# latentnetworks/vimure

Hardware: AMD Instinct MI355X
Metric: CAVI iterations/sec (L=4 N=2000 M=200 K=2 synthetic, mutuality on) (higher is better)
Workload: dtype f64

## Files before the change

### vimure_amd/csrc/sweep_sl.h

```cpp
#ifndef VMR_SWEEP_SL_H
#define VMR_SWEEP_SL_H

#include "vmr_internal.h"
#include <functional>

#define SL_YM(e) ((e) & 0xfffffu)
#define SL_INR(e) (((e) >> 20) & 1u)
#define SL_X(e) ((e) >> 21)
#define SL_XMAX 2047u
#define SL_YM_ROWS (1u << 20)
#define SL_PF 8
#ifndef SL_PFW
#define SL_PFW 8
#endif
constexpr int sl_pf(int K) { return K <= 2 ? SL_PF : SL_PFW; }
#define SL_SLACK (64 * 64)

struct SlArgs {
  const unsigned* E; const unsigned* rs; const unsigned long long* ebase; const unsigned* perm;
  const unsigned* sy;
  const uint8_t* cls;
  const unsigned* Qt;
  const uint64_t* Rb; const unsigned* rq; const unsigned short* Rm; const unsigned long long* rbase;
  const unsigned* rm2;
  double* rho; const double* logpr;
  const double* par; double* slotR; const double* lutg; double* Hg; double* slotF; double* slotA;
  int Gl;
  int do_hist;
  int yt, hc;
  int sum_a;
  double* nu_acc; double* elbo_dev; int commit_nu;
  int nu_stale;
  unsigned long long* det;
  int lp0;
  int farl;
  double* h0s;
  const unsigned* x0p;
  int lv0r;
  const unsigned* Ez;
  int elbo_cur;
  const double* lpd; const double* lpb;
#ifdef SL_DEBUG
  unsigned long long* dbg_t;
#endif
};

struct SlShape { int tpb, yt, hc; size_t smem; };
struct SlUnit { SlArgs a; Geo g; int blk0, nblk; };

#ifndef SL_LIGHT_UPD_K
#define SL_LIGHT_UPD_K 2
#endif
constexpr bool sl_light(int K, bool elbo, bool allfull, bool update) { return !elbo && allfull && (K <= SL_LIGHT_UPD_K || (!update && K <= 4)); }
#ifndef SL_ELBO3_K
#define SL_ELBO3_K 2
#endif
#ifndef SL_ELBO3
#define SL_ELBO3 1
#endif
constexpr int sl_tpb_max(int K, bool elbo, bool allfull, bool update = true) {
  return elbo ? ((SL_ELBO3 && K <= SL_ELBO3_K) ? 768 : (K <= 4 ? 512 : 256)) : (sl_light(K, elbo, allfull, update) ? 1024 : (K <= 3 ? 768 : (K <= 7 ? 512 : 256)));
}
constexpr int sl_tpb_max_b(int K, bool elbo, bool allfull) { return elbo ? sl_tpb_max(K, true, allfull) : (K <= 2 ? 768 : (K <= 7 ? 512 : 256)); }
constexpr int sl_wpe_b(int K, bool elbo, bool allfull) { return elbo ? ((SL_ELBO3 && K <= SL_ELBO3_K) ? 3 : (K <= 4 ? 2 : 1)) : (K <= 2 ? 3 : (K <= 7 ? 2 : 1)); }
constexpr int sl_wpe(int K, bool elbo, bool allfull, bool update = true) {
  return elbo ? ((SL_ELBO3 && K <= SL_ELBO3_K) ? 3 : (K <= 4 ? 2 : 1)) : (sl_light(K, elbo, allfull, update) ? 4 : (K <= 3 ? 3 : (K <= 7 ? 2 : 1)));
}

static inline size_t sl_smem(const Geo& g, int yt, int hc, bool update, bool elbo, bool hist) {
  const size_t lb = (size_t)g.Mp * g.K * 8;
  return (update ? (size_t)yt * lb : 0) + (hist ? (size_t)hc * lb : 0) + (size_t)g.Mp * 8 * (update ? 2 : 1) +
         (size_t)g.W * 8 + 128 + (g.ml ? lb + (size_t)g.Mp * 8 : 0) + (size_t)(64 + (elbo ? 256 : 0)) * 8 + 16;
}

typedef int (*sl_launch_fn)(vmr_ctx* h, int mode, const SlShape& sh, SlArgs& a);
sl_launch_fn vmr_sl_launcher(int K);
typedef int (*sl_launch_batch_fn)(vmr_ctx* h, hipStream_t st, int mode, int allfull, const SlUnit* units, const int* blk_unit, int nblocks,
                                  int tpb, size_t smem);
sl_launch_batch_fn vmr_sl_batch_launcher(int K);

#define SP_LDS_MAX (160 * 1024)
SlShape sl_shape(const vmr_ctx* h, bool update, bool elbo, bool hist);
SlArgs sl_args(const vmr_ctx* h, const SlShape& sh, int do_hist, int sum_a = 0);
int sl_launch(vmr_ctx* h, int mode, const SlShape& sh, SlArgs& a);

typedef std::function<void(int l, const unsigned* rpl, unsigned* etmp, unsigned* etmp2)> SlFill;
int sl_place_entries(vmr_ctx* h, unsigned* rp, const std::vector<unsigned long long>& nl, unsigned* etmp_all, unsigned* etmp2_all, const SlFill* fill);
int sl_balance_layer(vmr_ctx* h, int l, unsigned long long eb, unsigned rows_near);
int sl_permute_u8(vmr_ctx* h, const uint8_t* in, uint8_t* out);
int sl_permute_u32(vmr_ctx* h, const unsigned* in, unsigned* out);
int sl_permute_rows(vmr_ctx* h, const double* in, double* out, bool to_pos);

#endif
```

### vimure_amd/csrc/sweep_sl.hip

```cpp
#include "sweep_sl.h"

#ifndef VMR_K
#error "compile with -DVMR_K=<number of categories>"
#endif
#ifndef SL_WPE
#define SL_WPE sl_wpe(2, false, true)
#endif

template <int K>
struct StepIn {
  double v[K];
  double w[K];
  unsigned cls, qt, tie;
  unsigned x0;
  unsigned e[sl_pf(K)];
};

template <int R> struct RC { static constexpr int value = R; };
template <class V> __device__ __forceinline__ const V* at_bytes(const V* p, unsigned off) {
  return reinterpret_cast<const V*>(reinterpret_cast<const char*>(p) + off);
}
template <class V> __device__ __forceinline__ V* at_bytes(V* p, unsigned off) {
  return reinterpret_cast<V*>(reinterpret_cast<char*>(p) + off);
}
__device__ __forceinline__ double rcp_nr2(double d) {
  double r = __builtin_amdgcn_rcp(d);
  r = fma(fma(-d, r, 1.0), r, r);
  return fma(fma(-d, r, 1.0), r, r);
}
#define SL_INL __attribute__((always_inline))
#ifndef SL_BATCH2
#define SL_BATCH2 8
#endif
template <int K> struct Batch { static constexpr int value = K <= 2 ? SL_BATCH2 : (K <= 4 ? 4 : 2); };

template <int K, bool UPDATE, bool ELBO, bool ALLFULL, bool STORE = true, bool DET = false, bool LPD = false>
__device__ __forceinline__ void sweep_body(const SlArgs& a, const Geo& g, const unsigned bx, const unsigned gx) {
  extern __shared__ __align__(16) unsigned char smem[];
  constexpr int PFK = sl_pf(K);
  constexpr bool LV0 = !UPDATE && !ELBO && !DET;
  constexpr bool LV0R = UPDATE && K >= 3;
  const int tid = threadIdx.x, lane = tid & 63, nthr = (int)blockDim.x;
  const int wv = __builtin_amdgcn_readfirstlane(tid >> 6), nw = nthr >> 6;
  const int Mp = g.Mp;
  const unsigned ytm = UPDATE ? (unsigned)a.yt * (unsigned)Mp : 0u;
  const unsigned hcm = a.do_hist ? (unsigned)a.hc * (unsigned)Mp : 0u;
  size_t off = 0;
  double* F = reinterpret_cast<double*>(smem + off); off += (size_t)ytm * K * 8;
  const int nHc = (int)hcm * K;
  double* Hc = reinterpret_cast<double*>(smem + off); off += (size_t)nHc * 8;
  double* Gth = reinterpret_cast<double*>(smem + off); off += (size_t)Mp * 8;
  double* Lth = reinterpret_cast<double*>(smem + off); off += UPDATE ? (size_t)Mp * 8 : 0;
  double* As = reinterpret_cast<double*>(smem + off); off += a.sum_a ? (size_t)Mp * K * 8 : 0;
  double* wsum = reinterpret_cast<double*>(smem + off); off += (size_t)g.W * 8;
  double* red = reinterpret_cast<double*>(smem + off); off += 16 * 8;
  double* xt = reinterpret_cast<double*>(smem + off); off += 64 * 8;
  double* lt = reinterpret_cast<double*>(smem + off); off += ELBO ? 256 * 8 : 0;
  double* EthL = reinterpret_cast<double*>(smem + off); off += a.rq ? (size_t)Mp * 8 : 0;
  const ParOff o = par_off(g.L, g.Mp, g.K);
// ... 44 lines not shown
  unsigned long long ie_lin = 0ull, ie_q = 0ull, ie_log = 0ull, iaccF[K];
#pragma unroll
  for (int k = 0; k < K; ++k) iaccF[k] = 0ull;
  double* Hl = a.Hg + ((size_t)l * NH + (gb % NH)) * g.Y * Mp * K;
  auto det_H = [&]() SL_INL { return a.det + (size_t)l * g.Y * Mp * K; };
  auto det_A = [&]() SL_INL { return a.det + (size_t)g.L * g.Y * Mp * K + (size_t)l * g.W * 64 * K; };
  auto det_F = [&]() SL_INL { return a.det + (size_t)g.L * g.Y * Mp * K + (size_t)g.L * g.W * 64 * K + (size_t)l * K; };
  auto det_R = [&]() SL_INL { return a.det + (size_t)g.L * g.Y * Mp * K + (size_t)g.L * g.W * 64 * K + (size_t)g.L * K; };
  const unsigned* rsl = a.rs + (size_t)l * (NS + 1);
  const unsigned* syl = a.sy + (size_t)l * NS;
  const unsigned* El = a.E + a.ebase[l];
  const unsigned* pl = (a.rm2 ? a.rm2 : a.perm) + (size_t)l * NS * 64;
  const uint8_t* cl = ALLFULL ? nullptr : a.cls + (size_t)l * T;
  const unsigned* Ql = a.Qt ? a.Qt + (size_t)l * T : nullptr;
  const uint64_t* Rl = a.Rb ? a.Rb + (size_t)l * T * g.W : nullptr;
  double* rl = a.rho + (size_t)l * T * K;
  double* rho_slack = a.rho + (size_t)g.L * T * K;
  const double* lpl = a.logpr + (size_t)l * T * K;
  constexpr bool LPDV = LPD && K == 2 && UPDATE && !ELBO;
  const double* lpdl = LPDV ? a.lpd + (size_t)l * T : nullptr;
  const double lpb0 = (K == 2 && UPDATE) ? a.lpb[2 * l] : 0.0, lpb1 = (K == 2 && UPDATE) ? a.lpb[2 * l + 1] : 0.0;
  const unsigned* rql = a.rq ? a.rq + (size_t)l * (T + 1) : nullptr;
  const unsigned short* Rml = a.rq ? a.Rm + a.rbase[l] : nullptr;
  const unsigned lim_y = UPDATE ? (a.do_hist ? (unsigned)min(a.yt, a.hc) : (unsigned)a.yt) : (a.do_hist ? (unsigned)a.hc : 0xffffffffu);
  const unsigned lim1 = (UPDATE && a.yt < g.Y) ? (unsigned)a.yt : 0xffffffffu;
  const unsigned lim2 = (a.do_hist && a.hc < g.Y) ? (unsigned)a.hc : 0xffffffffu;

  const long long Gl_ = a.Gl;
  unsigned* tick = reinterpret_cast<unsigned*>(smem + off); off += 16;
  if (tid == 0) { tick[0] = 2u * (unsigned)nw; tick[1] = 0u; }
  auto step_of = [&](unsigned t) SL_INL -> long long { return (long long)gb + (long long)t * Gl_; };
  auto draw = [&]() SL_INL -> long long {
    unsigned t = 0u;
    if (lane == 0) t = atomicAdd(tick, 1u);
    return step_of((unsigned)__builtin_amdgcn_readfirstlane((int)t));
  };
  long long s = step_of((unsigned)wv), sn = step_of((unsigned)(nw + wv));
  unsigned ea = 0;
  int R = 0;
  unsigned ymax = 0;
  unsigned rgv = 0;
  StepIn<K> P;

  const unsigned lane4 = (unsigned)lane * 4u, laneK8 = (unsigned)lane * (unsigned)(K * 8);
  const unsigned T32 = (unsigned)T;
  auto fetch_range = [&](long long st) SL_INL {
    const unsigned ra = rsl[st + (lane < 1 ? 0 : 1)], ry = syl[st];
    rgv = lane == 2 ? ry : ra;
  };
  auto fetch_tie = [&](StepIn<K>& d, long long st, const bool lp_const = false) SL_INL {
    const size_t row0 = (size_t)st * 64;
    const bool ok = (unsigned)row0 + (unsigned)lane < T32;
    d.qt = 0u; d.tie = 0u;
// ... 31 lines not shown
    R = (int)((rsl[s + 1] - ea) >> 6);
    ymax = syl[s];
    fetch_range(sn < NS ? sn : s);
    fetch_tie(P, s);
    fetch_ent(P, ea, RC<PFK>{});
  }
#ifdef SL_DEBUG
  if (dbt && lane == 0) dbt[4] = wall_clock64();
#endif
  __builtin_amdgcn_s_waitcnt(0x0F70);
  bool lv0_off = false;
  if (LV0 || LV0R) lv0_off = __syncthreads_or(gz ? 1 : 0) != 0;
  else __syncthreads();
#ifdef SL_DEBUG
  if (dbt && lane == 0) dbt[5] = wall_clock64();
#endif
  const double gnu_f = a.par[o.sc + (a.nu_stale ? SC_G_NU_STALE : SC_G_NU)];
  if (UPDATE) {
    for (int q = tid; q < (int)ytm; q += nthr) {
      const int y = q / Mp, m = q - y * Mp;
#pragma unroll
      for (int k = 0; k < K; ++k) F[q * K + k] = (m < g.M) ? f_entry(g.mut, Lth[m], Gth[m], Lla[k], Gla[k], gnu_f, y) : 0.0;
    }
    __syncthreads();
  }
  double Tfull = 0.0;
  for (int w = 0; w < g.W; ++w) Tfull += wsum[w];
#ifdef SL_DEBUG
  if (dbt && lane == 0) dbt[1] = wall_clock64();
#endif

  auto add_lists = [&](unsigned t, bool on, const double (&rr)[K]) SL_INL {
    if (a.rm2) {
#pragma unroll
      for (int h_ = 0; h_ < 2; ++h_) {
        const unsigned m = h_ ? (t >> 16) : (t & 0xffffu);
        const bool v = on && m != 0xffffu;
        const unsigned long long vm = __ballot(v);
        if (vm == 0ull) continue;
        const int m0 = __builtin_amdgcn_readlane((int)m, __builtin_ctzll(vm));
        if (__all(!v || (int)m == m0)) {
#pragma unroll
          for (int k = 0; k < K; ++k) {
            const double sm_ = wave_sum(v ? rr[k] : 0.0);
            if (lane == 0) lds_add(&As[m0 * K + k], sm_, sc_a);
          }
        } else if (v) {
#pragma unroll
// ... 42 lines not shown
    }
    return Tt;
  };
  const double gnu_cur = a.par[o.sc + SC_G_NU];
  auto w2_at = [&](unsigned ym, int k) SL_INL -> double {
    const unsigned y = row_level(ym);
    const double z2 = gnu_cur * (double)y, den = Gth[ym - y * (unsigned)Mp] * Gla[k] + z2;
    return (y == 0u || den == 0.0) ? 0.0 : z2 / den;
  };
  auto f_far = [&](unsigned ym, double (&f)[K]) SL_INL {
    const unsigned y = row_level(ym);
    const unsigned m = ym - y * (unsigned)Mp;
    const double lt = Lth[m], gt = Gth[m];
#pragma unroll
    for (int k = 0; k < K; ++k) f[k] = f_entry(g.mut, lt, gt, Lla[k], Gla[k], gnu_f, (int)y);
  };
  auto elbo_inner = [&](unsigned ent, const double (&er)[2]) SL_INL -> double {
    const unsigned ym = SL_YM(ent);
    const unsigned y = row_level(ym);
    const double z2 = gnu * (double)y, gt = Gth[ym - y * (unsigned)Mp];
    const double inner = fma(gt, er[0], z2 * er[1]);
    return (SL_INR(ent) ? inner : 0.0) + eps;
  };
  auto walk1_near = [&](const unsigned* e, auto npc, double (&U)[K]) SL_INL {
    constexpr int NP = decltype(npc)::value, BT = Batch<K>::value;
#pragma unroll
    for (int j0 = 0; j0 < NP; j0 += BT) {
      double f[BT][K];
#pragma unroll
      for (int u = 0; u < BT; ++u) {
        if (j0 + u < NP) {
#pragma unroll
          for (int k = 0; k < K; ++k) f[u][k] = F[SL_YM(e[j0 + u]) * K + k];
        }
      }
#pragma unroll
      for (int u = 0; u < BT; ++u) {
        if (j0 + u < NP) {
          const double dx = (double)SL_X(e[j0 + u]);
#pragma unroll
          for (int k = 0; k < K; ++k) U[k] = fma(dx, f[u][k], U[k]);
        }
      }
    }
  };
  auto walk2_near = [&](const unsigned* e, auto npc, const double (&r)[K], const double (&er)[2]) SL_INL {
#ifndef SL_LG
#define SL_LG 2
#endif
    constexpr int NP = decltype(npc)::value, LG = SL_LG;
#pragma unroll
    for (int j0 = 0; j0 < NP; j0 += LG) {
      double in_[LG];
#pragma unroll
      for (int u = 0; u < LG; ++u) {
        if (j0 + u < NP) {
          const unsigned ym = SL_YM(e[j0 + u]);
          const double dx = (double)SL_X(e[j0 + u]);
          if (a.do_hist) {
#pragma unroll
            for (int k = 1; k < K; ++k) lds_add(&Hc[(unsigned)k * hcm + ym], dx * r[k], sc_h);
          }
          if (ELBO) in_[u] = elbo_inner(e[j0 + u], er);
        }
      }
      if (ELBO) {
#pragma unroll
        for (int u = 0; u < LG; ++u) if (j0 + u < NP) {
          const double term = (double)SL_X(e[j0 + u]) * log_tab(in_[u], lt);
          if (DET) ie_log += det_fx(term, g.det_shr); else e_log += term;
        }
        __builtin_amdgcn_sched_barrier(0);
      }
// ... 169 lines not shown
#pragma unroll
        for (int k = 0; k < K; ++k) { if (DET) iaccF[k] += fxm(r[k], sc_a); else accF[k] += r[k]; }
      }
      if (!ALLFULL && !ELBO && a.sum_a) add_lists(tie, act && cls == 2u, r);
    }
    if (ELBO) {
#pragma unroll
      for (int k = 0; k < K; ++k) { const double ek = exp_tab(r[k], xt); er[0] = fma(ek, Gla[k], er[0]); er[1] += ek; }
    }
#ifdef SL_DEBUG
    if (g.dbg & 32) {} else
#endif
    if (a.do_hist || ELBO) {
      if (RCT >= 0) {
        walk2_near(cur.e, RC<NP>{}, r, er);
        if (irr) {
#pragma unroll
          for (int j = 0; j < NP; ++j) deficit(cur.e[j], dfc);
        }
      } else {
        const bool skip0 = LV0 && a.x0p != nullptr && a.do_hist == 1 && n1 != 0x7fffffffu && !irr;
        const int Rw = skip0 ? min(Rr, (int)n1) : Rr;
        double sx0 = skip0 ? (double)cur.x0 : 0.0;
        rounds(RC<1>{}, [&](const unsigned (&c1)[1], const unsigned j) SL_INL {
          const unsigned c = c1[0], ym = SL_YM(c), x = SL_X(c);
          const bool far_round = j < nf && lim2 != 0xffffffffu;
          const bool fr = far_round && ym >= hcm;
          const double dx = (double)x;
          if (LV0 && a.do_hist && j >= n1) {
            sx0 += dx;
            if (irr) lds_add(&Hc[ym], dx * dfc, sc_h);
          } else if (a.do_hist) {
            if (!fr) {
              if (!(skip0 && ym < (unsigned)Mp)) {
#pragma unroll
                for (int k = 1; k < K; ++k) lds_add(&Hc[(unsigned)k * hcm + ym], dx * r[k], sc_h);
              }
              if (irr) lds_add(&Hc[ym], dx * dfc, sc_h);
            }
            if (far_round && !a.farl && __any(fr)) {
              if (fr && x != 0u) {
                if (DET) {
                  unsigned long long* d0 = a.det;
                  asm volatile("" : "+s"(d0));
                  unsigned long long* d = d0 + (size_t)l * g.Y * Mp * K + (size_t)ym * K;
#pragma unroll
                  for (int k = 1; k < K; ++k) atomicAdd(&d[k], fxm((double)x * r[k], sc_h));
                  if (dfc != 0.0) atomicAdd(&d[0], fxm((double)x * dfc, sc_h));
                } else {
                  double* d = Hl + (size_t)ym * K;
#pragma unroll
                  for (int k = 1; k < K; ++k) atomicAdd(&d[k], (double)x * r[k]);
                  if (dfc != 0.0) atomicAdd(&d[0], (double)x * dfc);
                }
              }
              asm volatile("" ::: "memory");
            }
          }
          if (ELBO) { const double term = (double)x * log_tab(elbo_inner(c, er), lt); if (DET) ie_log += det_fx(term, g.det_shr); else e_log += term; }
        }, Rw);
        if (LV0 && a.h0s && a.do_hist == 1 && act) {
#pragma unroll
          for (int k = 1; k < K; ++k) acc0[k] = fma(r[k], sx0, acc0[k]);
        }
      }
    }
    if (ELBO && act) {
      double sr = 0.0, se = 0.0, en = 0.0;
#pragma unroll
      for (int k = 0; k < K; ++k) {
        sr += r[k]; se += r[k] * Ela[k];
        en += r[k] * cur.v[k] - r[k] * log_tab(r[k] + eps, lt);
      }
      if (DET) { ie_lin += det_fx(en - se * Tt, g.det_shr); if (Ql) ie_q += det_fx(sr * (double)qt, g.det_shr); }
      else { e_lin += en - se * Tt; if (Ql) e_q += sr * (double)qt; }
    }
  };
  auto body = [&](auto rct) SL_INL {
    constexpr int RCT = decltype(rct)::value;
    constexpr int NP = RCT < 0 ? PFK : RCT;
    const size_t row0 = (size_t)s * 64;
    const bool act = (unsigned)row0 + (unsigned)lane < T32;
    const unsigned ea_c = ea;
// ... 197 lines not shown
    }
  }
  if (ELBO) {
    if (DET) {
      const unsigned long long v1 = wave_isum(ie_lin), v2 = wave_isum(ie_log), v3 = wave_isum(ie_q);
      if (lane == 0) { unsigned long long* dR = det_R(); atomicAdd(&dR[1], v1); atomicAdd(&dR[2], v2); atomicAdd(&dR[3], v3); }
    } else {
      double v1 = block_sum_n(e_lin, red);
      double v2 = block_sum_n(e_log, red);
      double v3 = block_sum_n(e_q, red);
      if (tid == 0) {
        double* out = a.slotR + (size_t)(bx % NSLOT) * 4;
        atomicAdd(&out[1], v1); atomicAdd(&out[2], v2); atomicAdd(&out[3], v3);
      }
    }
  }
#ifdef SL_DEBUG
  if (dbt && lane == 0) dbt[3] = wall_clock64();
#endif
}

#define SL_BOUNDS(K, UPDATE, ELBO, ALLFULL) \
  __launch_bounds__(sl_tpb_max(K, ELBO, ALLFULL, UPDATE), (K == 2 && !ELBO && ALLFULL) ? SL_WPE : sl_wpe(K, ELBO, ALLFULL, UPDATE))
template <int K, bool UPDATE, bool ELBO, bool ALLFULL, bool STORE = true, bool DET = false, bool LPD = false>
__global__ SL_BOUNDS(K, UPDATE, ELBO, ALLFULL) void k_sweep_sl(SlArgs a, Geo g) {
  sweep_body<K, UPDATE, ELBO, ALLFULL, STORE, DET, LPD>(a, g, blockIdx.x, gridDim.x);
}
template <int K, bool UPDATE, bool ELBO, bool ALLFULL, bool STORE = true, bool LPD = false>
__global__ __launch_bounds__(sl_tpb_max_b(K, ELBO, ALLFULL), sl_wpe_b(K, ELBO, ALLFULL)) void k_sweep_sl_b(const SlUnit* __restrict__ units, const int* __restrict__ blk_unit) {
  const SlUnit& u = units[blk_unit[blockIdx.x]];
  sweep_body<K, UPDATE, ELBO, ALLFULL, STORE, false, LPD>(u.a, u.g, blockIdx.x - (unsigned)u.blk0, (unsigned)u.nblk);
}

template <bool UPDATE, bool ELBO, bool ALLFULL, bool STORE = true, bool DET = false, bool LPD = false>
static int sl_launch_one_(vmr_ctx* h, const SlShape& sh, SlArgs& a) {
  constexpr int K = VMR_K;
  const Geo& g = h->g;
  const long long NS = ((long long)g.N * g.N + 63) / 64, nw = sh.tpb / 64;
  int rc = grid_per_layer(h, k_sweep_sl<K, UPDATE, ELBO, ALLFULL, STORE, DET, LPD>, sh.smem, &a.Gl, (NS + nw - 1) / nw, sh.tpb);
  if (rc) return rc;
#ifdef SL_DEBUG
  static unsigned long long* dbg_buf = nullptr;
  const char* tf = h->opt.debug_times[0] ? h->opt.debug_times : nullptr;
  const size_t nwv = (size_t)g.L * a.Gl * nw;
  a.dbg_t = nullptr;
  if (tf) {
    if (!dbg_buf) (void)hipMalloc(&dbg_buf, (size_t)1 << 22);
    if (nwv * 64 <= ((size_t)1 << 22)) a.dbg_t = dbg_buf;
  }
#endif
  hipLaunchKernelGGL((k_sweep_sl<K, UPDATE, ELBO, ALLFULL, STORE, DET, LPD>), dim3(g.L * a.Gl), dim3(sh.tpb), sh.smem, h->stream, a, g);
#ifdef SL_DEBUG
  if (a.dbg_t) {
    std::vector<unsigned long long> t(nwv * 8);
    (void)hipStreamSynchronize(h->stream);
    (void)hipMemcpy(t.data(), dbg_buf, nwv * 64, hipMemcpyDeviceToHost);
    if (FILE* f = fopen(tf, "a")) {
      fprintf(f, "launch %d%d hist %d waves %zu tpb %d\n", (int)UPDATE, (int)ELBO, a.do_hist, nwv, sh.tpb);
      for (size_t i = 0; i < nwv; ++i) fprintf(f, "%llu %llu %llu %llu %llu %llu %llu %llu\n", t[i * 8], t[i * 8 + 1], t[i * 8 + 2], t[i * 8 + 3], t[i * 8 + 4], t[i * 8 + 5], t[i * 8 + 6], t[i * 8 + 7]);
      fclose(f);
    }
  }
#endif
  return VMR_OK;
}

template <bool UPDATE, bool ELBO, bool ALLFULL, bool STORE = true, bool DET = false>
static int sl_launch_one(vmr_ctx* h, const SlShape& sh, SlArgs& a) {
  if (VMR_K == 2 && UPDATE && !ELBO && a.lpd) return sl_launch_one_<UPDATE, ELBO, ALLFULL, STORE, DET, VMR_K == 2 && UPDATE && !ELBO>(h, sh, a);
  return sl_launch_one_<UPDATE, ELBO, ALLFULL, STORE, DET>(h, sh, a);
}

#define SL_CAT2(a, b) a##b
#define SL_CAT(a, b) SL_CAT2(a, b)
int SL_CAT(vmr_sl_launch_k, VMR_K)(vmr_ctx* h, int mode, const SlShape& sh, SlArgs& a) {
  if (a.det) {
    if (a.cls == nullptr) {
      switch (mode) {
        case 0: return sl_launch_one<true, false, true, true, true>(h, sh, a);
        case 4: return sl_launch_one<true, false, true, false, true>(h, sh, a);
        case 1: return sl_launch_one<true, true, true, true, true>(h, sh, a);
        case 2: return sl_launch_one<false, true, true, true, true>(h, sh, a);
        default: return sl_launch_one<false, false, true, true, true>(h, sh, a);
      }
    }
    switch (mode) {
      case 0: return sl_launch_one<true, false, false, true, true>(h, sh, a);
      case 4: return sl_launch_one<true, false, false, false, true>(h, sh, a);
      case 1: return sl_launch_one<true, true, false, true, true>(h, sh, a);
      case 2: return sl_launch_one<false, true, false, true, true>(h, sh, a);
      default: return sl_launch_one<false, false, false, true, true>(h, sh, a);
    }
  }
  if (a.cls == nullptr) {
    switch (mode) {
      case 0: return sl_launch_one<true, false, true>(h, sh, a);
      case 1: return sl_launch_one<true, true, true>(h, sh, a);
      case 2: return sl_launch_one<false, true, true>(h, sh, a);
      case 4: return sl_launch_one<true, false, true, false>(h, sh, a);
      default: return sl_launch_one<false, false, true>(h, sh, a);
    }
  }
  switch (mode) {
    case 0: return sl_launch_one<true, false, false>(h, sh, a);
    case 1: return sl_launch_one<true, true, false>(h, sh, a);
    case 2: return sl_launch_one<false, true, false>(h, sh, a);
    case 4: return sl_launch_one<true, false, false, false>(h, sh, a);
    default: return sl_launch_one<false, false, false>(h, sh, a);
  }
}

template <bool UPDATE, bool ELBO, bool ALLFULL, bool STORE = true, bool LPD = false>
static int sl_launch_batch_one_(vmr_ctx* h, hipStream_t st, const SlUnit* units, const int* blk_unit, int nblocks, int tpb, size_t smem) {
  constexpr int K = VMR_K;
  if (smem > 48 * 1024)
    HIPCHK(h, hipFuncSetAttribute(reinterpret_cast<const void*>(k_sweep_sl_b<K, UPDATE, ELBO, ALLFULL, STORE, LPD>), hipFuncAttributeMaxDynamicSharedMemorySize, (int)smem));
  hipLaunchKernelGGL((k_sweep_sl_b<K, UPDATE, ELBO, ALLFULL, STORE, LPD>), dim3(nblocks), dim3(tpb), smem, st, units, blk_unit);
  return VMR_OK;
}
template <bool UPDATE, bool ELBO, bool ALLFULL, bool STORE = true>
static int sl_launch_batch_one(vmr_ctx* h, hipStream_t st, bool lpd, const SlUnit* units, const int* blk_unit, int nblocks, int tpb, size_t smem) {
  if (VMR_K == 2 && UPDATE && !ELBO && lpd) return sl_launch_batch_one_<UPDATE, ELBO, ALLFULL, STORE, VMR_K == 2 && UPDATE && !ELBO>(h, st, units, blk_unit, nblocks, tpb, smem);
  return sl_launch_batch_one_<UPDATE, ELBO, ALLFULL, STORE>(h, st, units, blk_unit, nblocks, tpb, smem);
}
int SL_CAT(vmr_sl_launch_batch_k, VMR_K)(vmr_ctx* h, hipStream_t st, int mode, int allfull, const SlUnit* units, const int* blk_unit, int nblocks,
                                          int tpb, size_t smem) {
  const bool lpd = h->lpd != nullptr;
  if (mode == 3) return allfull ? sl_launch_batch_one<false, false, true>(h, st, lpd, units, blk_unit, nblocks, tpb, smem)
                                : sl_launch_batch_one<false, false, false>(h, st, lpd, units, blk_unit, nblocks, tpb, smem);
  if (mode == 4) return allfull ? sl_launch_batch_one<true, false, true, false>(h, st, lpd, units, blk_unit, nblocks, tpb, smem)
                                : sl_launch_batch_one<true, false, false, false>(h, st, lpd, units, blk_unit, nblocks, tpb, smem);
  if (allfull) return mode ? sl_launch_batch_one<true, true, true>(h, st, lpd, units, blk_unit, nblocks, tpb, smem)
                           : sl_launch_batch_one<true, false, true>(h, st, lpd, units, blk_unit, nblocks, tpb, smem);
  return mode ? sl_launch_batch_one<true, true, false>(h, st, lpd, units, blk_unit, nblocks, tpb, smem)
              : sl_launch_batch_one<true, false, false>(h, st, lpd, units, blk_unit, nblocks, tpb, smem);
}
```

### vimure_amd/csrc/vimure_hip.hip

```cpp
#include "vmr_internal.h"
#include "sweep_sl.h"
#include "sweep_gen.h"
#include "sweep_tiles.h"
#include "create.h"
#include "sample_draw.h"

thread_local std::string g_create_err;

__global__ void k_init_rho(const double* __restrict__ pr, double* __restrict__ rho, double* __restrict__ logpr,
                           size_t n, double eps) {
  for (size_t q = blockIdx.x * (size_t)blockDim.x + threadIdx.x; q < n; q += (size_t)gridDim.x * blockDim.x) {
    double v = pr[q];
    rho[q] = v;
    logpr[q] = log(v + eps);
  }
}

__global__ void k_init_rho_pos(const double* __restrict__ pr, double* __restrict__ rho, double* __restrict__ logpr,
                               const unsigned* __restrict__ perm, size_t T, size_t NS, int L, int K, double eps,
                               const unsigned* __restrict__ rs, int* __restrict__ not_onehot) {
  const size_t n = (size_t)L * T * K;
  bool bad = false;
  for (size_t q = blockIdx.x * (size_t)blockDim.x + threadIdx.x; q < n; q += (size_t)gridDim.x * blockDim.x) {
    const size_t row = q / K, k = q - row * K, l = row / T, pos = row - l * T;
// ... 684 lines not shown
    }
  }
}


__global__ __launch_bounds__(256) void k_sample(const double* __restrict__ rho, uint8_t* __restrict__ out, size_t ties, int K, int n_trials,
                                                unsigned long long seed, const unsigned* __restrict__ perm, size_t T, size_t NS) {
  for (size_t q = (size_t)blockIdx.x * blockDim.x + threadIdx.x; q < ties; q += (size_t)gridDim.x * blockDim.x) {
    const double* r = rho + q * K;
    size_t t = q;
    if (perm) { const size_t l = q / T, pos = q - l * T; t = l * T + perm[l * NS * 64 + pos]; }
    const int best = draw_tie<false>(r, K, n_trials, seed, t, nullptr);
    out[t] = (uint8_t)best;
  }
}


SlShape sl_shape(const vmr_ctx* h, bool update, bool elbo, bool hist) {
  const Geo& g = h->g;
  SlShape s{std::max(64, std::min((update || elbo) ? h->sp_tpb : h->st_tpb, sl_tpb_max(g.K, elbo, h->all_full != 0, update)) & ~63), update ? g.yt : 0, hist ? g.hc : 0, 0};
  auto bytes = [&]() { return sl_smem(g, s.yt, s.hc, update, elbo, hist); };
  while (bytes() > SP_LDS_MAX && (s.yt > 0 || s.hc > 0)) { if (s.yt >= s.hc && s.yt > 0) --s.yt; else --s.hc; }
  s.smem = bytes();
  return s;
}
SlArgs sl_args(const vmr_ctx* h, const SlShape& sh, int do_hist, int sum_a) {
  return SlArgs{h->E, h->rs, h->ebase, h->perm, h->sy, h->cls_p, h->Qt_p, h->Rb, h->rq, h->Rm, h->rbase, h->rm2, h->rho, h->logpr, h->par, h->slotR,
                h->lutg, h->Hg, h->slotF, h->slotA, 1, do_hist, sh.yt, sh.hc, sum_a, nullptr, nullptr, 0, 0, nullptr, h->lp0 ? 1 : 0, h->g.farl, (do_hist == 1 && h->g.two_pass && sh.hc >= 1) ? h->h0s : nullptr, (do_hist == 1 && h->g.two_pass && sh.hc >= 1 && h->h0s) ? h->x0p : nullptr,
                (h->h0s && h->g.two_pass && !h->opt.no_lv0r) ? 1 : 0, h->E + h->n_slots, 0, h->lpd, h->lpb};
}
int sl_launch(vmr_ctx* h, int mode, const SlShape& sh, SlArgs& a) {
  sl_launch_fn fn = vmr_sl_launcher(h->g.K);
  if (!fn) return fail(h, VMR_EINVAL, "this build of libvimure_hip.so holds no sweep kernel for this K");
  return fn(h, mode, sh, a);
}

template <int K>
__global__ __launch_bounds__(1024) void k_far_hist(const unsigned* __restrict__ far_pos, const unsigned* __restrict__ far_ent,
                                                   const unsigned long long* __restrict__ fbase, const double* __restrict__ rho, double* Hg, double* par,
                                                   double* nu_acc, double* elbo_dev, int count, int commit_nu, int Gl, int LF, Geo g) {
  extern __shared__ double Hf[];
  const int Mp = g.Mp, tid = threadIdx.x, nthr = (int)blockDim.x;
  const int l = (int)blockIdx.x / Gl, gb = (int)blockIdx.x - l * Gl;
  const unsigned lfm = (unsigned)LF * (unsigned)Mp, hcm = (unsigned)g.hc * (unsigned)Mp;
  double* red = Hf + (size_t)K * lfm;
  for (unsigned q = tid; q < (unsigned)K * lfm; q += nthr) Hf[q] = 0.0;
  __syncthreads();
  const ParOff o = par_off(g.L, Mp, g.K);
  const size_t T = (size_t)g.N * g.N;
  double Gla[K];
#pragma unroll
  for (int k = 0; k < K; ++k) Gla[k] = par[o.G_la + l * K + k];
// ... 685 lines not shown
  if (rc) return rc;
  *n_rows = st.rows; *elbo_out = st.elbo; *iters_out = st.it - 1; *converged_out = st.reached;
  return VMR_OK;
}

static bool batch_steady(const vmr_ctx* h) {
  const Geo& g = h->g;
  return h->have_state && !h->restored && h->sparse && !g.two_pass && !g.farl && h->h_valid && !h->h_reduced && !h->h_zero &&
         h->f_valid == (g.fuse_full != 0) && (!g.ml || h->a_valid) && !h->prof;
}
static bool batch_kind(const vmr_ctx* h, const vmr_ctx* h0) {
  return h->sparse && !h->g.gen && !h->g.two_pass && !h->g.farl && !h->g.det && !h->prof && h->g.fuse_full && (h->n_partial == 0 || h->g.ml) && h->device == h0->device &&
         h->g.K == h0->g.K && h->g.mut == h0->g.mut && (h->all_full != 0) == (h0->all_full != 0) && !memcmp(&h->opt, &h0->opt, sizeof h->opt);
}
namespace {
struct BatchTables {
  SlUnit* su[3] = {nullptr, nullptr, nullptr};
  int* smap[3] = {nullptr, nullptr, nullptr};
  FinUnit* fu = nullptr;
  int *gmap = nullptr, *rmap = nullptr;
  double* be = nullptr;
  int nb[3] = {0, 0, 0}, ngb = 0, nrb = 0, tpb[3] = {0, 0, 0}, fg = FG_G;
  size_t smem[3] = {0, 0, 0}, fsm = 0;
  ~BatchTables() { for (void* p : {(void*)su[0], (void*)su[1], (void*)su[2], (void*)smap[0], (void*)smap[1], (void*)smap[2], (void*)fu, (void*)gmap, (void*)rmap, (void*)be}) if (p) (void)hipFree(p); }
};
}
static int batch_tables(vmr_ctx* const* hs, const std::vector<int>& act, int n_all, BatchTables& bt, hipStream_t st) {
  vmr_ctx* h0 = hs[act[0]];
  const int K = h0->g.K, allfull = h0->all_full != 0;
  long long steps = 0;
  for (int u : act) steps += (((long long)hs[u]->g.N * hs[u]->g.N + 63) / 64) * hs[u]->g.L;
  std::vector<FinUnit> fu(act.size());
  std::vector<int> gmap, rmap;
  for (int m = 0; m < 3; ++m) {
    const int tpb = sl_tpb_max_b(K, m == 1, allfull), nw = tpb / 64;
    long long per = std::max<long long>(4, std::min<long long>(64, (steps + (long long)nw * h0->ncu - 1) / ((long long)nw * h0->ncu)));
    {
      size_t smem_max = 0;
      for (int u : act) smem_max = std::max(smem_max, sl_shape(hs[u], m != 2, m == 1, true).smem);
      const int wpc = std::max<int>(1, std::min<int>((int)(SP_LDS_MAX / std::max<size_t>(smem_max, 1)), 4 * sl_wpe_b(K, m == 1, allfull) / nw));
      const long long cap_wgs = (long long)h0->ncu * wpc;
      auto total = [&](long long p_) {
        long long t = 0;
        for (int u : act) { const Geo& g = hs[u]->g; const long long NS = ((long long)g.N * g.N + 63) / 64; t += (long long)g.L * ((NS + nw * p_ - 1) / (nw * p_)); }
        return t;
      };
      if (total(per) > cap_wgs) {
        long long p2 = per;
        while (p2 < 512 && total(p2) > cap_wgs) p2 += std::max<long long>(1, p2 / 16);
        if (total(p2) <= cap_wgs) per = p2;
      }
    }
    std::vector<SlUnit> su(act.size());
    std::vector<int> map;
    size_t smem = 0;
    for (size_t i = 0; i < act.size(); ++i) {
      vmr_ctx* h = hs[act[i]];
      const Geo& g = h->g;
      const SlShape sh = sl_shape(h, m != 2, m == 1, true);
      SlArgs a = sl_args(h, sh, 1, g.ml ? 1 : 0);
      a.elbo_dev = bt.be + (size_t)act[i] * 8;
      if (g.mut && m != 2) { a.nu_acc = h->nu_acc; a.commit_nu = 1; }
      const long long NS = ((long long)g.N * g.N + 63) / 64;
      a.Gl = (int)std::max<long long>(1, std::min<long long>(4096, (NS + nw * per - 1) / (nw * per)));
      su[i].a = a; su[i].g = g; su[i].blk0 = (int)map.size(); su[i].nblk = g.L * a.Gl;
      map.insert(map.end(), (size_t)su[i].nblk, (int)i);
      smem = std::max(smem, sh.smem);
    }
    HIPCHK(h0, hipMemcpyAsync(bt.su[m], su.data(), su.size() * sizeof(SlUnit), hipMemcpyHostToDevice, st));
    HIPCHK(h0, hipMemcpyAsync(bt.smap[m], map.data(), map.size() * sizeof(int), hipMemcpyHostToDevice, st));
    HIPCHK(h0, hipStreamSynchronize(st));
    bt.nb[m] = (int)map.size(); bt.tpb[m] = tpb; bt.smem[m] = smem;
  }
  bt.fsm = 0;
  {
    long long layers = 0;
    for (int u : act) layers += hs[u]->g.L;
    bt.fg = (int)std::max<long long>(2, std::min<long long>(FG_G, (1LL * h0->ncu) / std::max<long long>(1, layers)));
    if (h0->opt.batch_fg) bt.fg = h0->opt.batch_fg;
  }
  for (size_t i = 0; i < act.size(); ++i) {
    vmr_ctx* h = hs[act[i]];
    const Geo& g = h->g;
    fu[i] = FinUnit{h->par, h->Hg, h->Cg, h->slotA, h->slotF, h->lutg, h->fin_g, h->nu_acc, h->slotR, bt.be + (size_t)act[i] * 8, g,
                    (int)gmap.size(), (int)rmap.size(), g.L * FR_G};
    gmap.insert(gmap.end(), (size_t)g.L * bt.fg, (int)i);
    rmap.insert(rmap.end(), (size_t)g.L * FR_G, (int)i);
    bt.fsm = std::max(bt.fsm, (size_t)2 * ((g.M + bt.fg - 1) / bt.fg) * 8);
  }
  HIPCHK(h0, hipMemcpyAsync(bt.fu, fu.data(), fu.size() * sizeof(FinUnit), hipMemcpyHostToDevice, st));
// ... 71 lines not shown
  BatchTables bt;
  {
    size_t blocks = 0, gb = 0, rb = 0;
    for (int u : act) {
      const Geo& g = hs[u]->g;
      blocks += (size_t)g.L * 4096; gb += (size_t)g.L * FG_G; rb += (size_t)g.L * FR_G;
    }
    for (int m = 0; m < 3; ++m) {
      HIPCHK(h0, hipMalloc(&bt.su[m], act.size() * sizeof(SlUnit)));
      HIPCHK(h0, hipMalloc(&bt.smap[m], blocks * sizeof(int)));
    }
    HIPCHK(h0, hipMalloc(&bt.fu, act.size() * sizeof(FinUnit)));
    HIPCHK(h0, hipMalloc(&bt.gmap, gb * sizeof(int)));
    HIPCHK(h0, hipMalloc(&bt.rmap, rb * sizeof(int)));
    HIPCHK(h0, hipMalloc(&bt.be, (size_t)n * 8 * 8));
    HIPCHK(h0, hipMemsetAsync(bt.be, 0, (size_t)n * 8 * 8, st));
  }
  std::vector<double> be_host((size_t)n * 8);
  int rc = batch_tables(hs, act, n, bt, st);
  if (rc) return rc;
  const bool lazy_rho = !h0->opt.always_store_rho;
  auto launch_sweeps = [&](int mode) -> int {
    hipLaunchKernelGGL(k_fin_gamma_b, dim3(bt.ngb), dim3(FIN_TPB), bt.fsm, st, bt.fu, bt.gmap, bt.fg);
    const int pm = (mode == 0 && lazy_rho) ? 4 : mode;
    int r = pass(h0, st, pm, allfull, bt.su[mode], bt.smap[mode], bt.nb[mode], bt.tpb[mode], bt.smem[mode]);
    for (int u : act) { hs[u]->rho_stale = pm == 4; hs[u]->prte_valid = false; }
    if (r) return r;
    if (mode == 1) hipLaunchKernelGGL(k_fin_rho_b, dim3(bt.nrb), dim3(TPB), 0, st, bt.fu, bt.rmap);
    HIPCHK(h0, hipGetLastError());
    return VMR_OK;
  };
  int it = fresh ? 1 : 2;
  while (!act.empty() && it <= max_iter) {
    const int nxt = (it == 1 || it % 10 == 0 || it == max_iter) ? it : std::min(max_iter, (it / 10 + 1) * 10);
    for (; it < nxt; ++it) if ((rc = launch_sweeps(0))) break;
    if (rc) break;
    HIPCHK(h0, hipStreamSynchronize(st));
    const auto t0 = std::chrono::steady_clock::now();
    if (it == 1) {
      for (int u : act) {
        vmr_ctx* h = hs[u];
        const Geo& g = h->g;
        HIPCHK(h0, hipMemsetAsync(h->Hg, 0, (size_t)g.L * NH * g.Y * g.Mp * g.K * 8, st));
        HIPCHK(h0, hipMemsetAsync(h->slotF, 0, (size_t)g.L * NSLOT * g.K * 8, st));
        if (g.ml) HIPCHK(h0, hipMemsetAsync(h->slotA, 0, (size_t)g.L * NSLOT * g.W * 64 * g.K * 8, st));
      }
      if ((rc = pass(h0, st, 3, allfull, bt.su[2], bt.smap[2], bt.nb[2], bt.tpb[2], bt.smem[2]))) break;
// ... 364 lines not shown
```

Before: 6307.

## Precompute ELBO inner-term table in LDS for K=2 sweeps

```diff
diff --git a/vimure_amd/csrc/sweep_sl.h b/vimure_amd/csrc/sweep_sl.h
--- a/vimure_amd/csrc/sweep_sl.h
+++ b/vimure_amd/csrc/sweep_sl.h
@@ -40,12 +40,13 @@
   const unsigned* Ez;
   int elbo_cur;
   const double* lpd; const double* lpb;
+  int ye;
 #ifdef SL_DEBUG
   unsigned long long* dbg_t;
 #endif
 };
 
-struct SlShape { int tpb, yt, hc; size_t smem; };
+struct SlShape { int tpb, yt, hc; size_t smem; int ye; };
 struct SlUnit { SlArgs a; Geo g; int blk0, nblk; };
 
 #ifndef SL_LIGHT_UPD_K
@@ -73,6 +74,9 @@
          (size_t)g.W * 8 + 128 + (g.ml ? lb + (size_t)g.Mp * 8 : 0) + (size_t)(64 + (elbo ? 256 : 0)) * 8 + 16;
 }
 
+constexpr bool sl_etab(int K) { return K == 2; }
+static inline size_t sl_smem_e(const Geo& g, int ye) { return ye > 0 ? (size_t)ye * g.Mp * 16 + 8 : 0; }
+
 typedef int (*sl_launch_fn)(vmr_ctx* h, int mode, const SlShape& sh, SlArgs& a);
 sl_launch_fn vmr_sl_launcher(int K);
 typedef int (*sl_launch_batch_fn)(vmr_ctx* h, hipStream_t st, int mode, int allfull, const SlUnit* units, const int* blk_unit, int nblocks,
diff --git a/vimure_amd/csrc/sweep_sl.hip b/vimure_amd/csrc/sweep_sl.hip
--- a/vimure_amd/csrc/sweep_sl.hip
+++ b/vimure_amd/csrc/sweep_sl.hip
@@ -32,9 +32,12 @@
 #ifndef SL_BATCH2
 #define SL_BATCH2 8
 #endif
+#ifndef SL_LGT
+#define SL_LGT 4
+#endif
 template <int K> struct Batch { static constexpr int value = K <= 2 ? SL_BATCH2 : (K <= 4 ? 4 : 2); };
 
-template <int K, bool UPDATE, bool ELBO, bool ALLFULL, bool STORE = true, bool DET = false, bool LPD = false>
+template <int K, bool UPDATE, bool ELBO, bool ALLFULL, bool STORE = true, bool DET = false, bool LPD = false, bool ETAB = false>
 __device__ __forceinline__ void sweep_body(const SlArgs& a, const Geo& g, const unsigned bx, const unsigned gx) {
   extern __shared__ __align__(16) unsigned char smem[];
   constexpr int PFK = sl_pf(K);
@@ -125,13 +128,18 @@
   const double lpb0 = (K == 2 && UPDATE) ? a.lpb[2 * l] : 0.0, lpb1 = (K == 2 && UPDATE) ? a.lpb[2 * l + 1] : 0.0;
   const unsigned* rql = a.rq ? a.rq + (size_t)l * (T + 1) : nullptr;
   const unsigned short* Rml = a.rq ? a.Rm + a.rbase[l] : nullptr;
-  const unsigned lim_y = UPDATE ? (a.do_hist ? (unsigned)min(a.yt, a.hc) : (unsigned)a.yt) : (a.do_hist ? (unsigned)a.hc : 0xffffffffu);
+  const unsigned lim_y0 = UPDATE ? (a.do_hist ? (unsigned)min(a.yt, a.hc) : (unsigned)a.yt) : (a.do_hist ? (unsigned)a.hc : 0xffffffffu);
+  constexpr bool ET = ETAB && ELBO && sl_etab(K);
+  const unsigned lim_y = ET ? min(lim_y0, (unsigned)a.ye) : lim_y0;
   const unsigned lim1 = (UPDATE && a.yt < g.Y) ? (unsigned)a.yt : 0xffffffffu;
   const unsigned lim2 = (a.do_hist && a.hc < g.Y) ? (unsigned)a.hc : 0xffffffffu;
 
   const long long Gl_ = a.Gl;
   unsigned* tick = reinterpret_cast<unsigned*>(smem + off); off += 16;
   if (tid == 0) { tick[0] = 2u * (unsigned)nw; tick[1] = 0u; }
+  off = (off + 15) & ~(size_t)15;
+  const unsigned yem = ET ? (unsigned)a.ye * (unsigned)Mp : 0u;
+  double2* Et = reinterpret_cast<double2*>(smem + off);
   auto step_of = [&](unsigned t) SL_INL -> long long { return (long long)gb + (long long)t * Gl_; };
   auto draw = [&]() SL_INL -> long long {
     unsigned t = 0u;
@@ -209,8 +217,14 @@
 #pragma unroll
       for (int k = 0; k < K; ++k) F[q * K + k] = (m < g.M) ? f_entry(g.mut, Lth[m], Gth[m], Lla[k], Gla[k], gnu_f, y) : 0.0;
     }
-    __syncthreads();
-  }
+  }
+  if (ET) {
+    for (int q = tid; q < (int)yem; q += nthr) {
+      const int y = q / Mp, m = q - y * Mp;
+      Et[q] = make_double2(Gth[m], gnu * (double)(unsigned)y);
+    }
+  }
+  if (UPDATE || ET) __syncthreads();
   double Tfull = 0.0;
   for (int w = 0; w < g.W; ++w) Tfull += wsum[w];
 #ifdef SL_DEBUG
@@ -299,6 +313,10 @@
     const double inner = fma(gt, er[0], z2 * er[1]);
     return (SL_INR(ent) ? inner : 0.0) + eps;
   };
+  auto elbo_inner_tab = [&](unsigned ent, const double2 ev, const double (&er)[2]) SL_INL -> double {
+    const double inner = fma(ev.x, er[0], ev.y * er[1]);
+    return ((ALLFULL || SL_INR(ent)) ? inner : 0.0) + eps;
+  };
   auto walk1_near = [&](const unsigned* e, auto npc, double (&U)[K]) SL_INL {
     constexpr int NP = decltype(npc)::value, BT = Batch<K>::value;
 #pragma unroll
@@ -326,6 +344,32 @@
 #define SL_LG 2
 #endif
     constexpr int NP = decltype(npc)::value, LG = SL_LG;
+    if (ET) {
+      constexpr int LGT = SL_LGT;
+      if (a.do_hist) {
+#pragma unroll
+        for (int j = 0; j < NP; ++j) {
+          const double dx = (double)SL_X(e[j]);
+#pragma unroll
+          for (int k = 1; k < K; ++k) lds_add(&Hc[(unsigned)k * hcm + SL_YM(e[j])], dx * r[k], sc_h);
+        }
+      }
+#pragma unroll
+      for (int j0 = 0; j0 < NP; j0 += LGT) {
+        double2 ev[LGT];
+#pragma unroll
+        for (int u = 0; u < LGT; ++u) if (j0 + u < NP) ev[u] = Et[SL_YM(e[j0 + u])];
+#pragma unroll
+        for (int u = 0; u < LGT; ++u) if (j0 + u < NP) {
+          const double term = (double)SL_X(e[j0 + u]) * log_tab(elbo_inner_tab(e[j0 + u], ev[u], er), lt);
+          if (DET) ie_log += det_fx(term, g.det_shr); else e_log += term;
+        }
+#ifdef SL_ESB
+        __builtin_amdgcn_sched_barrier(0);
+#endif
+      }
+      return;
+    }
 #pragma unroll
     for (int j0 = 0; j0 < NP; j0 += LG) {
       double in_[LG];
@@ -541,8 +585,8 @@
         const bool skip0 = LV0 && a.x0p != nullptr && a.do_hist == 1 && n1 != 0x7fffffffu && !irr;
         const int Rw = skip0 ? min(Rr, (int)n1) : Rr;
         double sx0 = skip0 ? (double)cur.x0 : 0.0;
-        rounds(RC<1>{}, [&](const unsigned (&c1)[1], const unsigned j) SL_INL {
-          const unsigned c = c1[0], ym = SL_YM(c), x = SL_X(c);
+        auto hist_entry = [&](const unsigned c, const unsigned j) SL_INL {
+          const unsigned ym = SL_YM(c), x = SL_X(c);
           const bool far_round = j < nf && lim2 != 0xffffffffu;
           const bool fr = far_round && ym >= hcm;
           const double dx = (double)x;
@@ -576,8 +620,35 @@
               asm volatile("" ::: "memory");
             }
           }
-          if (ELBO) { const double term = (double)x * log_tab(elbo_inner(c, er), lt); if (DET) ie_log += det_fx(term, g.det_shr); else e_log += term; }
-        }, Rw);
+        };
+        if (ET) {
+          constexpr int GE = SL_LGT;
+          rounds(RC<GE>{}, [&](const unsigned (&c)[GE], const unsigned j) SL_INL {
+#pragma unroll
+            for (int u = 0; u < GE; ++u) if (u == 0 || (int)(j + u) < Rw) hist_entry(c[u], j + (unsigned)u);
+            double2 ev[GE];
+            bool fr[GE];
+#pragma unroll
+            for (int u = 0; u < GE; ++u) {
+              const unsigned ym = SL_YM(c[u]);
+              fr[u] = ym >= yem;
+              ev[u] = Et[fr[u] ? 0u : ym];
+            }
+#pragma unroll
+            for (int u = 0; u < GE; ++u) {
+              double in_ = elbo_inner_tab(c[u], ev[u], er);
+              if (__any(fr[u])) { if (fr[u]) in_ = elbo_inner(c[u], er); }
+              const double term = (double)SL_X(c[u]) * log_tab(in_, lt);
+              if (DET) ie_log += det_fx(term, g.det_shr); else e_log += term;
+            }
+          }, Rw);
+        } else {
+          rounds(RC<1>{}, [&](const unsigned (&c1)[1], const unsigned j) SL_INL {
+            const unsigned c = c1[0];
+            hist_entry(c, j);
+            if (ELBO) { const double term = (double)SL_X(c) * log_tab(elbo_inner(c, er), lt); if (DET) ie_log += det_fx(term, g.det_shr); else e_log += term; }
+          }, Rw);
+        }
         if (LV0 && a.h0s && a.do_hist == 1 && act) {
 #pragma unroll
           for (int k = 1; k < K; ++k) acc0[k] = fma(r[k], sx0, acc0[k]);
@@ -821,22 +892,22 @@
 
 #define SL_BOUNDS(K, UPDATE, ELBO, ALLFULL) \
   __launch_bounds__(sl_tpb_max(K, ELBO, ALLFULL, UPDATE), (K == 2 && !ELBO && ALLFULL) ? SL_WPE : sl_wpe(K, ELBO, ALLFULL, UPDATE))
-template <int K, bool UPDATE, bool ELBO, bool ALLFULL, bool STORE = true, bool DET = false, bool LPD = false>
+template <int K, bool UPDATE, bool ELBO, bool ALLFULL, bool STORE = true, bool DET = false, bool LPD = false, bool ETAB = false>
 __global__ SL_BOUNDS(K, UPDATE, ELBO, ALLFULL) void k_sweep_sl(SlArgs a, Geo g) {
-  sweep_body<K, UPDATE, ELBO, ALLFULL, STORE, DET, LPD>(a, g, blockIdx.x, gridDim.x);
-}
-template <int K, bool UPDATE, bool ELBO, bool ALLFULL, bool STORE = true, bool LPD = false>
+  sweep_body<K, UPDATE, ELBO, ALLFULL, STORE, DET, LPD, ETAB>(a, g, blockIdx.x, gridDim.x);
+}
+template <int K, bool UPDATE, bool ELBO, bool ALLFULL, bool STORE = true, bool LPD = false, bool ETAB = false>
 __global__ __launch_bounds__(sl_tpb_max_b(K, ELBO, ALLFULL), sl_wpe_b(K, ELBO, ALLFULL)) void k_sweep_sl_b(const SlUnit* __restrict__ units, const int* __restrict__ blk_unit) {
   const SlUnit& u = units[blk_unit[blockIdx.x]];
-  sweep_body<K, UPDATE, ELBO, ALLFULL, STORE, false, LPD>(u.a, u.g, blockIdx.x - (unsigned)u.blk0, (unsigned)u.nblk);
-}
-
-template <bool UPDATE, bool ELBO, bool ALLFULL, bool STORE = true, bool DET = false, bool LPD = false>
+  sweep_body<K, UPDATE, ELBO, ALLFULL, STORE, false, LPD, ETAB>(u.a, u.g, blockIdx.x - (unsigned)u.blk0, (unsigned)u.nblk);
+}
+
+template <bool UPDATE, bool ELBO, bool ALLFULL, bool STORE = true, bool DET = false, bool LPD = false, bool ETAB = false>
 static int sl_launch_one_(vmr_ctx* h, const SlShape& sh, SlArgs& a) {
   constexpr int K = VMR_K;
   const Geo& g = h->g;
   const long long NS = ((long long)g.N * g.N + 63) / 64, nw = sh.tpb / 64;
-  int rc = grid_per_layer(h, k_sweep_sl<K, UPDATE, ELBO, ALLFULL, STORE, DET, LPD>, sh.smem, &a.Gl, (NS + nw - 1) / nw, sh.tpb);
+  int rc = grid_per_layer(h, k_sweep_sl<K, UPDATE, ELBO, ALLFULL, STORE, DET, LPD, ETAB>, sh.smem, &a.Gl, (NS + nw - 1) / nw, sh.tpb);
   if (rc) return rc;
 #ifdef SL_DEBUG
   static unsigned long long* dbg_buf = nullptr;
@@ -848,7 +919,7 @@
     if (nwv * 64 <= ((size_t)1 << 22)) a.dbg_t = dbg_buf;
   }
 #endif
-  hipLaunchKernelGGL((k_sweep_sl<K, UPDATE, ELBO, ALLFULL, STORE, DET, LPD>), dim3(g.L * a.Gl), dim3(sh.tpb), sh.smem, h->stream, a, g);
+  hipLaunchKernelGGL((k_sweep_sl<K, UPDATE, ELBO, ALLFULL, STORE, DET, LPD, ETAB>), dim3(g.L * a.Gl), dim3(sh.tpb), sh.smem, h->stream, a, g);
 #ifdef SL_DEBUG
   if (a.dbg_t) {
     std::vector<unsigned long long> t(nwv * 8);
@@ -867,6 +938,7 @@
 template <bool UPDATE, bool ELBO, bool ALLFULL, bool STORE = true, bool DET = false>
 static int sl_launch_one(vmr_ctx* h, const SlShape& sh, SlArgs& a) {
   if (VMR_K == 2 && UPDATE && !ELBO && a.lpd) return sl_launch_one_<UPDATE, ELBO, ALLFULL, STORE, DET, VMR_K == 2 && UPDATE && !ELBO>(h, sh, a);
+  if (sl_etab(VMR_K) && ELBO && a.ye > 0) return sl_launch_one_<UPDATE, ELBO, ALLFULL, STORE, DET, false, sl_etab(VMR_K) && ELBO>(h, sh, a);
   return sl_launch_one_<UPDATE, ELBO, ALLFULL, STORE, DET>(h, sh, a);
 }
 
@@ -909,12 +981,12 @@
   }
 }
 
-template <bool UPDATE, bool ELBO, bool ALLFULL, bool STORE = true, bool LPD = false>
+template <bool UPDATE, bool ELBO, bool ALLFULL, bool STORE = true, bool LPD = false, bool ETAB = false>
 static int sl_launch_batch_one_(vmr_ctx* h, hipStream_t st, const SlUnit* units, const int* blk_unit, int nblocks, int tpb, size_t smem) {
   constexpr int K = VMR_K;
   if (smem > 48 * 1024)
-    HIPCHK(h, hipFuncSetAttribute(reinterpret_cast<const void*>(k_sweep_sl_b<K, UPDATE, ELBO, ALLFULL, STORE, LPD>), hipFuncAttributeMaxDynamicSharedMemorySize, (int)smem));
-  hipLaunchKernelGGL((k_sweep_sl_b<K, UPDATE, ELBO, ALLFULL, STORE, LPD>), dim3(nblocks), dim3(tpb), smem, st, units, blk_unit);
+    HIPCHK(h, hipFuncSetAttribute(reinterpret_cast<const void*>(k_sweep_sl_b<K, UPDATE, ELBO, ALLFULL, STORE, LPD, ETAB>), hipFuncAttributeMaxDynamicSharedMemorySize, (int)smem));
+  hipLaunchKernelGGL((k_sweep_sl_b<K, UPDATE, ELBO, ALLFULL, STORE, LPD, ETAB>), dim3(nblocks), dim3(tpb), smem, st, units, blk_unit);
   return VMR_OK;
 }
 template <bool UPDATE, bool ELBO, bool ALLFULL, bool STORE = true>
@@ -927,6 +999,9 @@
   const bool lpd = h->lpd != nullptr;
   if (mode == 3) return allfull ? sl_launch_batch_one<false, false, true>(h, st, lpd, units, blk_unit, nblocks, tpb, smem)
                                 : sl_launch_batch_one<false, false, false>(h, st, lpd, units, blk_unit, nblocks, tpb, smem);
+  if (mode == 5 && sl_etab(VMR_K))
+    return allfull ? sl_launch_batch_one_<true, true, true, true, false, sl_etab(VMR_K)>(h, st, units, blk_unit, nblocks, tpb, smem)
+                   : sl_launch_batch_one_<true, true, false, true, false, sl_etab(VMR_K)>(h, st, units, blk_unit, nblocks, tpb, smem);
   if (mode == 4) return allfull ? sl_launch_batch_one<true, false, true, false>(h, st, lpd, units, blk_unit, nblocks, tpb, smem)
                                 : sl_launch_batch_one<true, false, false, false>(h, st, lpd, units, blk_unit, nblocks, tpb, smem);
   if (allfull) return mode ? sl_launch_batch_one<true, true, true>(h, st, lpd, units, blk_unit, nblocks, tpb, smem)
diff --git a/vimure_amd/csrc/vimure_hip.hip b/vimure_amd/csrc/vimure_hip.hip
--- a/vimure_amd/csrc/vimure_hip.hip
+++ b/vimure_amd/csrc/vimure_hip.hip
@@ -730,12 +730,20 @@
   auto bytes = [&]() { return sl_smem(g, s.yt, s.hc, update, elbo, hist); };
   while (bytes() > SP_LDS_MAX && (s.yt > 0 || s.hc > 0)) { if (s.yt >= s.hc && s.yt > 0) --s.yt; else --s.hc; }
   s.smem = bytes();
+  s.ye = 0;
+  if (elbo && sl_etab(g.K)) {
+    const int lv = update ? (hist ? std::min(s.yt, s.hc) : s.yt) : (hist ? s.hc : g.Y);
+    const size_t with = s.smem + sl_smem_e(g, lv);
+    const int nw = s.tpb / 64, wcu = 4 * sl_wpe(g.K, true, h->all_full != 0, update);
+    auto resident = [&](size_t b) { return std::min<long long>((long long)(SP_LDS_MAX / b), std::max(1, wcu / nw)); };
+    if (lv > 0 && with + 64 <= SP_LDS_MAX && resident(with) >= resident(s.smem)) { s.ye = lv; s.smem = with; }
+  }
   return s;
 }
 SlArgs sl_args(const vmr_ctx* h, const SlShape& sh, int do_hist, int sum_a) {
   return SlArgs{h->E, h->rs, h->ebase, h->perm, h->sy, h->cls_p, h->Qt_p, h->Rb, h->rq, h->Rm, h->rbase, h->rm2, h->rho, h->logpr, h->par, h->slotR,
                 h->lutg, h->Hg, h->slotF, h->slotA, 1, do_hist, sh.yt, sh.hc, sum_a, nullptr, nullptr, 0, 0, nullptr, h->lp0 ? 1 : 0, h->g.farl, (do_hist == 1 && h->g.two_pass && sh.hc >= 1) ? h->h0s : nullptr, (do_hist == 1 && h->g.two_pass && sh.hc >= 1 && h->h0s) ? h->x0p : nullptr,
-                (h->h0s && h->g.two_pass && !h->opt.no_lv0r) ? 1 : 0, h->E + h->n_slots, 0, h->lpd, h->lpb};
+                (h->h0s && h->g.two_pass && !h->opt.no_lv0r) ? 1 : 0, h->E + h->n_slots, 0, h->lpd, h->lpb, sh.ye};
 }
 int sl_launch(vmr_ctx* h, int mode, const SlShape& sh, SlArgs& a) {
   sl_launch_fn fn = vmr_sl_launcher(h->g.K);
@@ -1467,6 +1475,7 @@
   double* be = nullptr;
   int nb[3] = {0, 0, 0}, ngb = 0, nrb = 0, tpb[3] = {0, 0, 0}, fg = FG_G;
   size_t smem[3] = {0, 0, 0}, fsm = 0;
+  bool etab = false;
   ~BatchTables() { for (void* p : {(void*)su[0], (void*)su[1], (void*)su[2], (void*)smap[0], (void*)smap[1], (void*)smap[2], (void*)fu, (void*)gmap, (void*)rmap, (void*)be}) if (p) (void)hipFree(p); }
 };
 }
@@ -1499,10 +1508,12 @@
     std::vector<SlUnit> su(act.size());
     std::vector<int> map;
     size_t smem = 0;
+    bool all_e = m == 1;
     for (size_t i = 0; i < act.size(); ++i) {
       vmr_ctx* h = hs[act[i]];
       const Geo& g = h->g;
       const SlShape sh = sl_shape(h, m != 2, m == 1, true);
+      all_e = all_e && sh.ye > 0;
       SlArgs a = sl_args(h, sh, 1, g.ml ? 1 : 0);
       a.elbo_dev = bt.be + (size_t)act[i] * 8;
       if (g.mut && m != 2) { a.nu_acc = h->nu_acc; a.commit_nu = 1; }
@@ -1511,6 +1522,10 @@
       su[i].a = a; su[i].g = g; su[i].blk0 = (int)map.size(); su[i].nblk = g.L * a.Gl;
       map.insert(map.end(), (size_t)su[i].nblk, (int)i);
       smem = std::max(smem, sh.smem);
+    }
+    if (m == 1) {
+      bt.etab = all_e;
+      if (!all_e) for (SlUnit& u_ : su) u_.a.ye = 0;
     }
     HIPCHK(h0, hipMemcpyAsync(bt.su[m], su.data(), su.size() * sizeof(SlUnit), hipMemcpyHostToDevice, st));
     HIPCHK(h0, hipMemcpyAsync(bt.smap[m], map.data(), map.size() * sizeof(int), hipMemcpyHostToDevice, st));
@@ -1628,7 +1643,7 @@
   const bool lazy_rho = !h0->opt.always_store_rho;
   auto launch_sweeps = [&](int mode) -> int {
     hipLaunchKernelGGL(k_fin_gamma_b, dim3(bt.ngb), dim3(FIN_TPB), bt.fsm, st, bt.fu, bt.gmap, bt.fg);
-    const int pm = (mode == 0 && lazy_rho) ? 4 : mode;
+    const int pm = (mode == 0 && lazy_rho) ? 4 : (mode == 1 && bt.etab) ? 5 : mode;
     int r = pass(h0, st, pm, allfull, bt.su[mode], bt.smap[mode], bt.nb[mode], bt.tpb[mode], bt.smem[mode]);
     for (int u : act) { hs[u]->rho_stale = pm == 4; hs[u]->prte_valid = false; }
     if (r) return r;
```

Result: no change. 6292 (median of 2 runs) (-0.2%).
